# GadGadGad/Convolutional-KAN-for-Image-Classification

Hardware: AMD Instinct MI355X
Metric: images/sec fwd+bwd KAN-VGG11 3x32x32 bs=256/GPU (higher is better)
Workload: dtype f32

## Files before the change

convolutional-kan-for-image-classification_amd/_lib.py:

```python
from __future__ import annotations

import ctypes as C
import os
from typing import Optional

_HERE = os.path.dirname(os.path.abspath(__file__))
LIB_PATH = os.environ.get("KANCONV_LIB") or os.path.join(_HERE, "libkanconv.so")

KAN_MAX_PLANES = 16
KAN_MAX_TABLE = 32
KAN_FP_WORDS = 192
BASIS_BSPLINE, BASIS_RBF, BASIS_CHEBY, BASIS_POLY, BASIS_FOURIER, BASIS_RELU, BASIS_GRAM = 0, 1, 2, 3, 4, 5, 6
ACT_NONE, ACT_IDENTITY, ACT_GELU, ACT_SILU, ACT_RELU, ACT_TANH, ACT_SIGMOID, ACT_GELU_TANH = -1, 0, 1, 2, 3, 4, 5, 6


class KanGeom(C.Structure):
    _fields_ = [(n, C.c_int) for n in ("B", "C", "H", "W", "O", "Ho", "Wo", "kh", "kw", "sh", "sw", "ph", "pw", "dh", "dw", "groups")] + \
               [("x_bstride", C.c_longlong), ("y_bstride", C.c_longlong)]


class KanBasis(C.Structure):
    _fields_ = [("kind", C.c_int), ("n_basis", C.c_int), ("order", C.c_int), ("act", C.c_int),
                ("p0", C.c_float), ("p1", C.c_float), ("table", C.c_float * KAN_MAX_TABLE), ("chan_table", C.c_void_p)]


class KanPlan(C.Structure):
    _fields_ = [(n, C.c_int) for n in ("P", "K", "IPC", "KC", "Kpad", "Opad", "fwd_splits", "bwd_data_splits", "bwd_weight_splits",
                                          "fwd_target", "bwd_data_target", "bwd_weight_target", "x_pm_wanted", "dz_pm_wanted", "bwd_weight_expanded", "row_blocks", "e_pm_wanted", "fwd_expanded", "fwd_halo", "bwd_weight_halo",
                                          "fwd_band", "bwd_weight_band")] + \
               [(n, C.c_longlong) for n in ("packed_weight_bytes", "bwd_data_weight_bytes", "fwd_slab_elems", "bwd_data_slab_elems",
                                            "bwd_weight_slab_elems", "e_pm_elems")]


class KanWavGeom(C.Structure):
    _fields_ = [(n, C.c_int) for n in ("B", "C", "H", "W", "O", "Ho", "Wo", "kh", "kw", "sh", "sw", "ph", "pw", "dh", "dw", "wavelet")] + \
               [("x_bstride", C.c_longlong), ("u_bstride", C.c_longlong)]


WAVELETS = {"mexican_hat": 0, "morlet": 1, "dog": 2, "meyer": 3, "shannon": 4}

_P, _I, _LL, _F, _D = C.c_void_p, C.c_int, C.c_longlong, C.c_float, C.c_double
_GP, _BP = C.POINTER(KanGeom), C.POINTER(KanBasis)
SIGNATURES = {
    "kan_version": (C.c_char_p, []),
    "kan_last_error": (C.c_char_p, []),
    "kan_plan": (_I, [_GP, _BP, C.POINTER(KanPlan)]),
    "kan_pack_weights": (_I, [_P, _P, _P, _P, _GP, _BP, _P]),
    "kan_pack_cacheable": (_I, [_GP, _BP]),
    "kan_pack_weights_cached": (_I, [_P, _P, _P, _P, _GP, _BP, _P, _I, _I, _I, _P]),
    "kan_conv_fwd": (_I, [_P, _P, _P, _P, _GP, _BP, _P, _P]),
    "kan_position_major": (_I, [_P, _P, _I, _I, _I, _LL, _P]),
    "kan_conv_bwd_data": (_I, [_P, _P, _P, _P, _P, _P, _GP, _BP, _P, _P]),
    "kan_conv_bwd_data_params": (_I, [_P, _P, _P, _P, _P, _P, _P, _GP, _BP, _P, _P]),
    "kan_conv_bwd_weight": (_I, [_P, _P, _P, _P, _GP, _BP, _P, _P, _P]),
    "kan_position_major_expanded": (_I, [_P, _P, _GP, _BP, _P]),
    "kan_conv_fwd_expanded": (_I, [_P, _P, _P, _GP, _BP, _P]),
    "kan_conv_bwd_weight_expanded": (_I, [_P, _P, _P, _GP, _BP, _P]),
    "kan_unpack_wgrad": (_I, [_P, _P, _P, _GP, _BP, _P]),
    "kan_slab_reduce": (_I, [_P, _I, _LL, _P, _I, _I, _I, _LL, _P]),
    "kan_instnorm_prelu_fwd": (_I, [_P, _I, _LL, _P, _P, _P, _P, _P, _P, _P, _I, _I, _I, _LL, _F, _I, _P]),
    "kan_instnorm_prelu_bwd": (_I, [_P, _P, _P, _P, _P, _P, _P, _P, _P, _P, _P, _I, _I, _I, _LL, _I, _P]),
    "kan_instnorm_prelu_pool_fwd": (_I, [_P, _I, _LL, _P, _P, _P, _P, _P, _P, _P, _P, _I, _I, _I, _I, _LL, _F, _I, _P]),
    "kan_instnorm_prelu_pool_bwd": (_I, [_P, _P, _P, _P, _P, _P, _P, _P, _P, _P, _P, _P, _I, _I, _I, _I, _LL, _I, _P]),
    "kan_instnorm_prelu_poolk_fwd": (_I, [_P, _I, _LL, _P, _P, _P, _P, _P, _P, _P, _P, _I, _I, _I, _I, _LL, _F, _I, _I, _I, _P]),
    "kan_instnorm_prelu_poolk_bwd": (_I, [_P, _P, _P, _P, _P, _P, _P, _P, _P, _P, _P, _P, _I, _I, _I, _I, _LL, _I, _I, _I, _P]),
    "kan_split_supported": (_I, [C.POINTER(KanGeom), C.POINTER(KanBasis)]),
    "kan_split_weight_bytes": (_LL, [C.POINTER(KanGeom), C.POINTER(KanBasis)]),
    "kan_split_pack_weights": (_I, [_P, _P, _P, C.POINTER(KanGeom), C.POINTER(KanBasis), _P]),
    "kan_conv_fwd_split": (_I, [_P, _P, _P, C.POINTER(KanGeom), C.POINTER(KanBasis), _P]),
    "kan_wav_fwd": (_I, [_P, _P, _P, _P, _P, C.POINTER(KanWavGeom), _P]),
    "kan_wav_bwd_input": (_I, [_P, _P, _P, _P, _P, _P, C.POINTER(KanWavGeom), _P]),
    "kan_wav_param_workspace": (_LL, [C.POINTER(KanWavGeom)]),
    "kan_wav_bwd_params": (_I, [_P, _P, _P, _P, _P, _P, _P, _P, _P, C.POINTER(KanWavGeom), _P]),
    "kan_adamw_step": (_I, [_P, _P, _P, _P, _LL, _D, _D, _D, _D, _D, _I, _F, _P]),
    "kan_adamw_step_segments": (_I, [_P, _P, _P, _P, _P, _P, _P, _P, _P, _I, _I, _D, _D, _D, _D, _D, _I, _F, _P]),
}

_lib: Optional[C.CDLL] = None

# ... 29 lines not shown
```

convolutional-kan-for-image-classification_amd/csrc/kan_internal.h:

```cpp
#pragma once
#include <type_traits>
#include "kanconv.h"

int kan_fail_msg(const char* fmt, const char* a);
int kan_raise_lds_limit(const void* kernel, int bytes);

enum : int {
    FAST_GENERIC = 0,
    FAST_BSPLINE_SILU = 1,
    FAST_BSPLINE_GELU = 2,
    FAST_RBF8 = 3,
    FAST_CHEBY5 = 4,
    FAST_CHEBY4 = 5,
    FAST_POLY4 = 6,
    FAST_POLY3 = 7,
    FAST_RBF5 = 8,
    FAST_RELU8 = 9,
    FAST_GRAM4 = 10,
    FAST_POLY1 = 11,
    FAST_LAST = 11
};
enum : unsigned {
    ON_TAP_MAJOR = 1u << 0,
    ON_BIG_TILES = 1u << 1,
    ON_HALO_FWD = 1u << 2,
    ON_HALO_BWD_WEIGHT = 1u << 3,
    ON_BAND_FWD = 1u << 4,
    ON_BAND_BWD_WEIGHT = 1u << 5,
    ON_EXPANDED_FWD = 1u << 6,
    ON_EXPANDED = 1u << 7,
    ON_ROWBLK_BWD_DATA = 1u << 8,
};
struct FastSpec {
    int kind, planes;
    bool base;
    bool xn_fwd, xn_bwd;
    int kc;
    unsigned routes;
};
constexpr FastSpec fast_spec(int f) {
    constexpr unsigned bspline = ON_TAP_MAJOR | ON_BIG_TILES | ON_HALO_FWD | ON_HALO_BWD_WEIGHT | ON_BAND_FWD | ON_BAND_BWD_WEIGHT |
                                 ON_EXPANDED_FWD | ON_EXPANDED | ON_ROWBLK_BWD_DATA;
    switch (f) {
        case FAST_BSPLINE_SILU: case FAST_BSPLINE_GELU: return {KAN_BASIS_BSPLINE, 9, true, false, false, 18, bspline};
        case FAST_RBF8: return {KAN_BASIS_RBF, 9, true, true, true, 18, ON_TAP_MAJOR | ON_BAND_FWD | ON_BAND_BWD_WEIGHT};
        case FAST_RBF5: return {KAN_BASIS_RBF, 6, true, true, true, 18, ON_TAP_MAJOR};
        case FAST_CHEBY5: return {KAN_BASIS_CHEBY, 5, false, false, false, 16, ON_TAP_MAJOR | ON_BIG_TILES | ON_BAND_FWD | ON_BAND_BWD_WEIGHT};
        case FAST_CHEBY4: return {KAN_BASIS_CHEBY, 4, false, false, false, 16, ON_TAP_MAJOR | ON_HALO_FWD | ON_BAND_FWD};
        case FAST_POLY4: return {KAN_BASIS_POLY, 5, true, true, false, 16, ON_TAP_MAJOR | ON_BIG_TILES | ON_HALO_FWD | ON_BAND_FWD};
        case FAST_POLY3: return {KAN_BASIS_POLY, 4, true, true, false, 16, ON_TAP_MAJOR};
        case FAST_POLY1: return {KAN_BASIS_POLY, 2, true, true, false, 16, ON_TAP_MAJOR};
        case FAST_RELU8: return {KAN_BASIS_RELU, 9, true, false, false, 16, ON_HALO_FWD | ON_HALO_BWD_WEIGHT | ON_EXPANDED_FWD | ON_EXPANDED};
        case FAST_GRAM4: return {KAN_BASIS_GRAM, 5, true, false, false, 16, ON_HALO_FWD | ON_HALO_BWD_WEIGHT | ON_EXPANDED};
        default: return {-1, 0, false, true, true, 0, 0};
    }
}
constexpr int fast_kind(int f) { return fast_spec(f).kind; }
constexpr int fast_planes(int f) { return fast_spec(f).planes; }
constexpr bool fast_has(int f, unsigned routes) { return (fast_spec(f).routes & routes) == routes && f != FAST_GENERIC; }

template <int V> using IC = std::integral_constant<int, V>;
template <unsigned ROUTES, int F = 1, class Fn>
bool dispatch_fast(int f, Fn&& fn) {
    if constexpr (F > FAST_LAST) {
        return false;
    } else {
        if constexpr (fast_has(F, ROUTES)) {
            if (f == F) { fn(IC<F>{}); return true; }
        }
        return dispatch_fast<ROUTES, F + 1>(f, fn);
    }
}
template <int V, int... REST, class Fn>
void pick(int v, Fn&& fn) {
    if constexpr (sizeof...(REST) == 0) fn(IC<V>{});
// ... 21 lines not shown
    int lds_bytes, wgs_per_cu;
    int fwd_splits;
    int bw_ok, bw_WR, bw_NI, bw_NT, bw_tiles_o, bw_row_tiles, bw_TPI, bw_ptiles, bw_cells, bw_slots, bw_lds_bytes, bw_splits;
    unsigned short bw_ph_rt0[KAN_BAND_MAX_PHASES + 1];
    unsigned char ph_a[KAN_BAND_MAX_PHASES], ph_b[KAN_BAND_MAX_PHASES];
    short ph_tap0[KAN_BAND_MAX_PHASES + 1];
    unsigned short tap_shift[KAN_BAND_MAX_TAPS];
    unsigned short tap_rt[KAN_BAND_MAX_TAPS];
    short tap_step[KAN_BAND_MAX_TAPS], tap_nt[KAN_BAND_MAX_TAPS];
} KanBandCfg;

void kan_band_cfg(const KanGeom* g, const KanBasis* b, int fast, KanBandCfg* cfg);
int kan_band_bwd_weight_launch(const float* dz, const float* x, const float* xn, float* dwp, const KanGeom* g, const KanBasis* b,
                               const KanBandCfg* cfg, int splits, long long slab_elems, void* stream);
int kan_band_fwd_launch(const float* x, const float* xn, const float* wp, float* z, const KanGeom* g, const KanBasis* b,
                        const KanBandCfg* cfg, int splits, long long slab_elems, void* stream);

constexpr int DW_T = 9;
constexpr int DW_MAX_TP = 96;

enum class Route { TAP_MAJOR, DW, BAND, HALO, EXPANDED };

struct FwdCfg { int TO, TP, tiles_o, tiles_p, chunks, splits, slots; };
struct BdCfg { int CH, tiles_c, tiles_p, n_ob, Opad32, chunks, splits; };
struct BwCfg { int TR, TO, tiles_r, tiles_o, chunks, splits, slots; };
struct BwHaloCfg { int R, nimg, spb, n_bands, tiles_r, tiles_o, splits, bands_per_split; };

struct ConvPlan {
    KanPlan pub;
    int fast;
    Route fwd, bwd_data, bwd_weight;
    bool pm_fwd, pm_bwd_data, pm_bwd_weight;
    bool rowblk_bwd_data;
    bool pmdma_xcd, pm_lpt, pm_xcd;
    FwdCfg fc;
    BdCfg bd;
    BwCfg bw;
    BwHaloCfg bwh;
    KanBandCfg band;
};
int plan_conv(const KanGeom* g, const KanBasis* b, ConvPlan* cp);

int live_taps_out(const KanGeom* g, int hw);
int live_taps_in(const KanGeom* g, int hw);
int live_positions_for_tap(const KanGeom* g, int tap);
int balance_tiles(const int* weight, int n, unsigned short* idx);
```

convolutional-kan-for-image-classification_amd/csrc/kan_plan.hip:

```cpp
#include <hip/hip_runtime.h>
#include <cstdio>
#include <cstdlib>
#include <cstring>
#include "kanconv.h"
#include "kan_device.h"
#include "kan_common.h"
#include "kan_internal.h"

namespace {

int fail(const char* msg) { return kan_fail_msg("%s", msg); }

int check(const KanGeom* g, const KanBasis* b) {
    if (!g || !b) return fail("null geometry/basis");
    if (g->groups < 0 || g->groups > 65535) return fail("groups out of range");
    if (g->B <= 0 || g->C <= 0 || g->O <= 0 || g->H <= 0 || g->W <= 0 || g->Ho <= 0 || g->Wo <= 0) return fail("non-positive dimension");
    if (g->kh <= 0 || g->kw <= 0 || g->sh <= 0 || g->sw <= 0 || g->dh <= 0 || g->dw <= 0 || g->ph < 0 || g->pw < 0) return fail("bad conv parameters");
    if (g->kh > 255 || g->kw > 255 || g->C > 65535) return fail("kernel size / channel count out of supported range");
    if ((g->H + 2 * g->ph - g->dh * (g->kh - 1) - 1) / g->sh + 1 != g->Ho || (g->W + 2 * g->pw - g->dw * (g->kw - 1) - 1) / g->sw + 1 != g->Wo)
        return fail("Ho/Wo inconsistent with H/W, kernel, stride, padding, dilation");
    if ((long long)g->B * g->Ho * g->Wo >= (1ll << 31) || (long long)g->B * g->H * g->W >= (1ll << 31)) return fail("pixel count exceeds int32");
    if ((long long)g->B * g->x_bstride * 4 >= (1ll << 31) || (long long)g->B * g->y_bstride * 4 >= (1ll << 31))
        return fail("activation tensors must be smaller than 2 GiB (32-bit buffer offsets)");
    if (g->x_bstride < (long long)ngroups(g) * g->C * g->H * g->W || g->y_bstride < (long long)ngroups(g) * g->O * g->Ho * g->Wo)
// ... 94 lines not shown
    if (g->kh != 3 || g->kw != 3 || g->sh != 1 || g->sw != 1 || g->dh != 1 || g->dw != 1 || g->ph != 1 || g->pw != 1) return false;
    if ((g->C & 1) || g->O % 128 != 0) return false;
    if (pm_fwd) return false;
    const int W = g->W, H = g->H;
    return (W == 32 && H % 4 == 0) || (W == 16 && H % 8 == 0) || (W == 8 && H == 8) || (W == 4 && H == 4);
}
bool band_fwd(const KanGeom* g, const KanBasis* b, int f, bool dw, bool pm_fwd, bool halo, KanBandCfg* out) {
    if (tuning_off("KAN_BAND") || !fast_has(f, ON_BAND_FWD)) return false;
    if (b->kind == KAN_BASIS_POLY && b->order == 0) return false;
    if (dw || pm_fwd || halo) return false;
    if (!(g->C <= 3 || round_up(g->O, 64) % 128 != 0 || (g->kh * g->kw >= 4 && g->C % 2 == 0 && !tuning_off("KAN_BAND_WIDE")))) return false;
    kan_band_cfg(g, b, f, out);
    return out->ok != 0;
}
FwdCfg fwd_cfg(const KanGeom* g, const KanPlan& pl, bool big, bool pm_fwd, bool halo) {
    FwdCfg c;
    c.TO = (big && !pm_fwd) ? 256 : (pl.Opad % 128 == 0) ? 128 : 64;
    c.slots = c.TO == 256 ? 512 : 1024;
    c.TP = 128;
    c.tiles_o = pl.Opad / c.TO;
    c.tiles_p = ceil_div((long long)g->B * g->Ho * g->Wo, c.TP);
    c.chunks = pl.Kpad / pl.KC;
    c.splits = pick_splits((long long)c.tiles_o * c.tiles_p * ngroups(g), c.chunks, 8, 4.0 * g->B * g->O * g->Ho * g->Wo * ngroups(g), c.slots);
    if (halo) {
        const int n_pairs = g->C / 2, pps = ceil_div(n_pairs, c.splits < n_pairs ? c.splits : n_pairs);
        c.splits = ceil_div(n_pairs, pps);
    }
    return c;
}
bool rowblk_bwd_data(const KanGeom* g, int f, bool pm_bwd_data) {
    return !tuning_off("KAN_BD_ROWBLK") && fast_has(f, ON_ROWBLK_BWD_DATA) && !pm_bwd_data && g->H == 4 && g->W == 4 && g->Ho == 4 && g->Wo == 4 &&
           g->kh == 3 && g->kw == 3 && g->sh == 1 && g->sw == 1 && g->ph == 1 && g->pw == 1 && g->dh == 1 && g->dw == 1 && g->B % 8 == 0 && g->O % 16 == 0;
}
struct LiveClass { long long tiles; int live_steps; };

int pick_target_steps(const LiveClass* cls, int ncls, int min_steps, double slab_bytes, int* max_splits, long long SLOTS = 1024) {
    int hi = 1;
    for (int i = 0; i < ncls; ++i) if (cls[i].live_steps > hi) hi = cls[i].live_steps;
    int best = hi; double best_cost = -1; int best_ms = 1;
    for (int t = min_steps < hi ? min_steps : hi; t <= hi; ++t) {
        long long wgs = 0; int ms = 1;
        for (int i = 0; i < ncls; ++i) {
            const int sp = cls[i].live_steps > 0 ? ceil_div(cls[i].live_steps, t) : 1;
            wgs += cls[i].tiles * sp;
            if (sp > ms) ms = sp;
        }
        const long long rounds = (wgs + SLOTS - 1) / SLOTS;
        const double cost = (double)(rounds * (t + 6)) + ms * slab_cost_steps(slab_bytes);
        if (best_cost < 0 || cost < best_cost) { best_cost = cost; best = t; best_ms = ms; }
    }
    *max_splits = best_ms;
    return best;
}
BdCfg bd_cfg(const KanGeom* g, const KanPlan& pl) {
    BdCfg c;
    c.CH = 64 / pl.P;
    c.tiles_c = ceil_div(g->C, 2 * c.CH);
    c.tiles_p = ceil_div((long long)g->B * g->H * g->W, 128);
    c.n_ob = ceil_div(g->O, 16);
    c.Opad32 = round_up(g->O, 32);
    c.chunks = g->kh * g->kw * c.n_ob;
    c.splits = pick_splits((long long)c.tiles_c * c.tiles_p * ngroups(g), c.chunks, 8, 4.0 * g->B * g->C * g->H * g->W * ngroups(g));
    return c;
}
bool pmdma_bwd_weight(const KanGeom* g, const KanBasis* b, int f, bool want_pm_bw) {
    if (tuning_off("KAN_PMDMA") || !fast_has(f, ON_EXPANDED)) return false;
// ... 98 lines not shown
        order[j] = v;
    }
    for (int r = 0; r < n; ++r) {
        const int depth = r / 8, k = r % 8, bin = (depth & 1) ? 7 - k : k;
        int slot = depth * 8 + bin;
        if (slot >= n) slot = r;
        idx[slot] = (unsigned short)order[r];
    }
    bool seen[PERM_MAX] = {false};
    for (int i = 0; i < n; ++i) { if (idx[i] >= n || seen[idx[i]]) return 0; seen[idx[i]] = true; }
    return n;
}

int plan_conv(const KanGeom* g, const KanBasis* b, ConvPlan* cp) {
    if (int rc = check(g, b)) return rc;
    ConvPlan& c = *cp;
    KanPlan* pl = &c.pub;
    const int T = g->kh * g->kw, G = ngroups(g), f = fast_variant(b);
    c.fast = f;
    const bool pm_shape = pmdma_fwd_shape(g, f);
    c.pm_fwd = want_pix_major(g, b, PM_FWD, pm_shape);
    c.pm_bwd_data = want_pix_major(g, b, PM_BWD_DATA, false);
    const bool want_pm_bw = want_pix_major(g, b, PM_BWD_WEIGHT, false);
    const bool dw = dw_direct(g, b);
    const bool halo = halo_fwd(g, b, f, c.pm_fwd);
    c.band.ok = c.band.bw_ok = 0;
    const bool band = band_fwd(g, b, f, dw, c.pm_fwd, halo, &c.band);
    const bool pmdma_fwd = pm_shape && c.pm_fwd;
    const bool pmdma_bw = pmdma_bwd_weight(g, b, f, want_pm_bw);
    const bool halo_bw = halo_bwd_weight(g, f, pmdma_bw);
    c.pm_bwd_weight = want_pm_bw && !halo_bw;
    const bool band_bw = band && c.band.bw_ok && !want_pm_bw && !tuning_off("KAN_BAND_BW");
    c.rowblk_bwd_data = rowblk_bwd_data(g, f, c.pm_bwd_data);
    c.pmdma_xcd = tuning_on("KAN_PMDMA_XCD");
    c.pm_lpt = !tuning_off("KAN_PM_LPT");
    c.pm_xcd = !tuning_off("KAN_PM_XCD");
    c.fwd = dw ? Route::DW : band ? Route::BAND : halo ? Route::HALO : pmdma_fwd ? Route::EXPANDED : Route::TAP_MAJOR;
    c.bwd_data = dw ? Route::DW : Route::TAP_MAJOR;
    c.bwd_weight = dw ? Route::DW : band_bw ? Route::BAND : halo_bw ? Route::HALO : pmdma_bw ? Route::EXPANDED : Route::TAP_MAJOR;
    pl->P = b->n_basis + (b->act != KAN_ACT_NONE);
    pl->K = g->C * T * pl->P;
    {
        int i18 = 18 / pl->P, i16 = 16 / pl->P;
        if (i18 > 4) i18 = 4;
        if (i16 > 4) i16 = 4;
        const bool use18 = (long long)i18 * pl->P * 16 > (long long)i16 * pl->P * 18;
        pl->KC = use18 ? 18 : 16;
        pl->IPC = use18 ? i18 : i16;
        if (pl->P >= 10 && pl->P <= 12) { pl->KC = 12; pl->IPC = 1; }
        if (halo) { pl->KC = 2 * pl->P; pl->IPC = 2; }
    }
    pl->Kpad = ceil_div(g->C * T, pl->IPC) * pl->KC;
    if (band) { pl->KC = c.band.NPLE; pl->IPC = c.band.NG; pl->Kpad = c.band.n_steps * c.band.NPLE; }
    pl->Opad = round_up(g->O, 64);
    pl->packed_weight_bytes = (long long)G * pl->Kpad * pl->Opad * 4;
    c.bd = bd_cfg(g, *pl);
    pl->bwd_data_weight_bytes = (long long)G * T * c.bd.Opad32 * c.bd.tiles_c * 128 * 4;
    pl->fwd_slab_elems = (long long)g->B * g->y_bstride;
    pl->bwd_data_slab_elems = (long long)g->B * g->x_bstride;
    pl->bwd_weight_slab_elems = (long long)G * pl->K * pl->Opad;
    const bool big = big_tiles(f, *pl);
    c.fc = fwd_cfg(g, *pl, big, c.pm_fwd, halo);
    c.bw = bw_cfg(g, *pl, big, c.pm_bwd_weight);
    if (halo_bw) c.bwh = bw_halo_cfg(g, *pl);
    pl->fwd_splits = band ? c.band.fwd_splits : c.fc.splits;
    pl->bwd_data_splits = c.bd.splits;
// ... 45 lines not shown
```

convolutional-kan-for-image-classification_amd/csrc/kanconv.hip:

```cpp
#include <hip/hip_runtime.h>
#include <cstdio>
#include <cstdlib>
#include <cstring>
#include <cmath>
#include <cstdint>
#include <mutex>
#include <type_traits>
#include <vector>
#include "kanconv.h"
#include "kan_device.h"

#include "kan_common.h"
#include "kan_internal.h"

namespace {


thread_local char g_err[512] = "";
int fail(const char* fmt, const char* a = "") {
    snprintf(g_err, sizeof(g_err), fmt, a);
    return -1;
}
}
int kan_fail_msg(const char* fmt, const char* a) { return fail(fmt, a); }
// ... 557 lines not shown
            for (int r = 0; r < 16; ++r) {
                const int o = o_tile0 + w_o * 64 + mi * 32 + mfma_row(r, lane);
                if (o < g.O) zb[(size_t)o * HoWo] = acc[mi][ni][r];
            }
        }
    }
}

template <int M>
__device__ __forceinline__ void wave_reduce_scatter(float (&v)[M], int lane, int& idx, float& tot) {
    int base = 0;
    int m = M;
#pragma unroll
    for (int off = 32; off >= 1; off >>= 1) {
        if (m > 1) {
            const int h = m / 2;
            const bool up = (lane & off) != 0;
#pragma unroll
            for (int i = 0; i < M / 2; ++i) {
                if (i < h) {
                    const float keep = up ? v[h + i] : v[i], send = up ? v[i] : v[h + i];
                    v[i] = keep + __shfl_xor(send, off, 64);
                }
            }
            base += up ? h : 0;
            m = h;
        } else {
            v[0] += __shfl_xor(v[0], off, 64);
        }
    }
    idx = base; tot = v[0];
}

template <int KIND, int FAST, int RB = 0>
__global__ __launch_bounds__(256, 4) void k_conv_bwd_data(
    const float* __restrict__ dz, const float* __restrict__ x, const float* __restrict__ xn, const float* __restrict__ wd,
    float* __restrict__ dx, float* __restrict__ dxn, DevGeom g, DevBasis bs, int CH, int n_ct, int n_ob, int Opad16,
    int n_chunks, int chunks_per_split, long long slab_elems, unsigned dz_bytes, TilePerm perm, float* __restrict__ dpar) {
    constexpr int TP = 128, KD = 16, NT = 256;
    __shared__ __attribute__((aligned(16))) float smem[2 * 2 * KD * 128];
    __shared__ float sTab[KAN_MAX_TABLE];

    const int tid = threadIdx.x, lane = tid & 63;
    const int wave = __builtin_amdgcn_readfirstlane(tid >> 6);
    const int w_r = wave >> 1, w_p = wave & 1;
    const int HoWo = g.Ho * g.Wo, HW = g.H * g.W, P = bs.P;
    const int Min = g.B * HW;
    const BlockId blk = xcd_block_order(false);
    const int grp = blk.y / n_ct;
    const int px_tile0 = (perm.n ? (int)perm.idx[blk.x] : blk.x) * TP, ct = blk.y - grp * n_ct;
    const int ncol = n_ct * 128;
    const int pxl = (wave & 1) * 64 + lane, ol0 = wave >> 1;
    const bool idle_rows = (ct * 2 + w_r) * CH >= g.C;
    {
        const size_t xo = (size_t)grp * g.C * HW;
        x += xo; xn += xo; dx += xo; if (dxn) dxn += xo;
        dz += (size_t)grp * g.O * HoWo * (g.pix_major ? g.B : 1);
        wd += (size_t)grp * (g.kh * g.kw) * Opad16 * ncol;
    }

    if (tid < KAN_MAX_TABLE) sTab[tid] = bs.tab[tid];
    const int my_px = px_tile0 + (RB ? ((pxl >> 2) & 7) * 16 + (pxl >> 5) * 4 + (pxl & 3) : pxl);
    const bool pv = my_px < Min;
    int pb, ph_, pw_;
    {
        int hw;
        if (g.pix_major) { hw = my_px / g.B; pb = my_px - hw * g.B; }
        else { pb = my_px / HW; hw = my_px - pb * HW; }
        ph_ = hw / g.W; pw_ = hw - ph_ * g.W;
    }
    const kan_rsrc dz_rs = make_rsrc(dz, dz_bytes);
    const unsigned dz_img = g.pix_major ? (unsigned)pb : (unsigned)pb * (unsigned)g.ybs;
    const unsigned zstride = g.pix_major ? (unsigned)g.B : 1u;
// ... 86 lines not shown
    for (int a = 0; a < 2; ++a)
#pragma unroll
        for (int b = 0; b < 2; ++b)
#pragma unroll
            for (int r = 0; r < 16; ++r) acc[a][b][r] = 0.f;

    int ch0 = blk.z * chunks_per_split;
    int ch1 = min(n_chunks, ch0 + chunks_per_split);
    unsigned tapmask = 0xffffffffu;
    if (g.pix_major) {
        tapmask = 0;
        const int T = g.kh * g.kw;
        const int hwA = px_tile0 / g.B, hwB = min(px_tile0 + TP - 1, Min - 1) / g.B;
        for (int hw = hwA; hw <= hwB; ++hw)
            for (int tap = 0; tap < T; ++tap) tapmask |= (tap_alive_in(g, hw, tap) ? 1u : 0u) << tap;
        auto seg = [&](int tap) { return tap * n_ob; };
        const int L = live_step_count(tapmask, T, n_chunks, seg);
        const int S = min((int)gridDim.z, max(1, (L + chunks_per_split - 1) / chunks_per_split));
        if (blk.z >= S) { ch0 = ch1 = n_chunks; }
        else {
            ch0 = blk.z == 0 ? 0 : live_step_pos(tapmask, T, n_chunks, (int)((long long)L * blk.z / S), seg);
            ch1 = blk.z == S - 1 ? n_chunks : live_step_pos(tapmask, T, n_chunks, (int)((long long)L * (blk.z + 1) / S), seg);
        }
    }
    auto next_live = [&](int ch) -> int {
        if (!g.pix_major) return ch;
        while (ch < ch1) {
            const int tap = ch / n_ob;
            if ((tapmask >> tap) & 1u) return ch;
            ch = (tap + 1) * n_ob;
        }
        return ch1;
    };
    int ch = next_live(ch0);
    if (ch < ch1) { if (RB) issue_rb(ch, 0); else issue(ch, 0); }
    const int ar = w_r * 64 + (lane & 31), bp = w_p * 64 + (lane & 31), kh2 = lane >> 5;
    for (int cur = 0; ch < ch1; cur ^= 1) {
        asm volatile("s_waitcnt vmcnt(0)" ::: "memory");
        __syncthreads();
        const bool mixed_now = pend_mixed;
        ch = next_live(ch + 1);
        if (ch < ch1) { if (RB) issue_rb(ch, cur ^ 1); else issue(ch, cur ^ 1); }
        const float* cW = smem + cur * (2 * KD * 128);
        const float* cG = cW + KD * 128;
        const unsigned aw = lds_addr(cW + kh2 * 128 + ar), ag = lds_addr(cG + kh2 * TP + bp);
        if (RB) {
            const bool l0b = !(mixed_now && w_p == 0), l1a = !(mixed_now && w_p == 1);
            if (!idle_rows) KAN_MFMA_STEP_LIVE(KD / 2, aw, 128, ag, TP, true, l0b, l1a, true);
        } else if (!idle_rows) KAN_MFMA_STEP(KD / 2, aw, 128, ag, TP);
    }

    const bool same_in = (x == xn);
    const bool split_out = (dxn != nullptr);
    float* dxs = dx + (size_t)blk.z * slab_elems;
    float* dxns = split_out ? dxn + (size_t)blk.z * slab_elems : nullptr;
#define KAN_G_TO_LDS(half)                                                                                                 \
    __syncthreads();                                                                                                       \
    if (w_r == (half)) {                                                                                                   \
        _Pragma("unroll") for (int mi = 0; mi < 2; ++mi)                                                                   \
            _Pragma("unroll") for (int ni = 0; ni < 2; ++ni)                                                               \
                _Pragma("unroll") for (int r = 0; r < 16; ++r)                                                             \
                    smem[(mi * 32 + mfma_row(r, lane)) * TP + w_p * 64 + ni * 32 + (lane & 31)] = acc[mi][ni][r];          \
    }                                                                                                                      \
    __syncthreads();
    if constexpr (FAST != 0) {
        constexpr FastSpec S = fast_spec(FAST);
        constexpr int FP = S.planes, FCH = 64 / FP, NIT = (FCH + 1) / 2, NPF = S.xn_bwd ? 1 : 2;
        float xv[NPF][NIT], nv[NIT]; unsigned ok = 0;
#define KAN_FETCH(half, slot)                                                                                              \
        _Pragma("unroll") for (int it = 0; it < NIT; ++it) {                                                                   \
            const int cl = ol0 + 2 * it, c = (ct * 2 + (half)) * FCH + cl;                                                     \
            const bool v = cl < FCH && c < g.C && pv;                                                                          \
            const size_t idx = (size_t)pb * g.xbs + (size_t)c * HW + (size_t)(ph_ * g.W + pw_);                                \
            xv[slot][it] = v ? x[idx] : 0.f;                                                                                   \
            if constexpr (S.xn_bwd) nv[it] = v ? xn[idx] : 0.f;                                                                \
            ok |= (v ? 1u : 0u) << ((slot) * NIT + it);                                                                        \
        }
        if constexpr (!S.xn_bwd) {
#pragma unroll
            for (int half = 0; half < 2; ++half) KAN_FETCH(half, half)
        }
#pragma unroll 1
// ... 1440 lines not shown
        const int t = (n & ~3) + threadIdx.x;
        if (t < n) adam1(p[t], g[t], m[t], v[t], a);
    } else {
        for (int i = threadIdx.x; i < n; i += 256) adam1(p[i], g[i], m[i], v[i], a);
    }
}

AdamArgs adam_args(double lr, double beta1, double beta2, double eps, double weight_decay, int step, float grad_scale) {
    const double bc1 = 1.0 - pow(beta1, (double)step), bc2 = 1.0 - pow(beta2, (double)step);
    AdamArgs a;
    a.decay = (float)(1.0 - lr * weight_decay);
    a.w1 = (float)(1.0 - beta1); a.b2 = (float)beta2; a.w2 = (float)(1.0 - beta2);
    a.gscale = grad_scale; a.inv_bc2_sqrt = (float)(1.0 / sqrt(bc2)); a.eps = (float)eps; a.neg_step = (float)(-lr / bc1);
    return a;
}

#include "wavkan.inc"

}

extern "C" {

const char* kan_version(void) { return "kanconv 0.5 (gfx950, fp32 MFMA 32x32x2, halo forward, 128/256-output tiles)"; }
const char* kan_last_error(void) { return g_err; }

int kan_plan(const KanGeom* geom, const KanBasis* basis, KanPlan* plan) {
    if (!plan) return fail("null plan");
    ConvPlan cp;
    if (int rc = plan_conv(geom, basis, &cp)) return rc;
    *plan = cp.pub;
    return 0;
}

static bool pack_needs_clear(const KanGeom* g, const KanPlan& pl) {
    if (pl.fwd_band) return pl.KC != pl.IPC * pl.P || g->C % pl.IPC != 0;
    return pl.KC != pl.IPC * pl.P || (g->C * g->kh * g->kw) % pl.IPC != 0;
}

static int pack_weights_impl(const float* w_base, const float* w_basis, float* wp, float* wd, const KanGeom* g, const KanBasis* b,
                             const unsigned long long* fp, int fp_cur, void* stream) {
    ConvPlan cp;
    if (int rc = plan_conv(g, b, &cp)) return rc;
    const KanPlan& pl = cp.pub;
    const int hb = b->act != KAN_ACT_NONE;
    if ((hb && !w_base) || !w_basis || !wp) return fail("null weight pointer");
    hipStream_t st = (hipStream_t)stream;
    const int T = g->kh * g->kw, NI = g->C * T, G = ngroups(g);
    const long long wp_gs = (long long)pl.Kpad * pl.Opad;
    PackGeo q = pack_geo(g, b, cp, false);
    if (fp && (pack_needs_clear(g, pl) || cp.fwd == Route::DW)) return fail("cached packing is not offered for this geometry (kan_pack_cacheable)");
    if (pl.KC != pl.IPC * pl.P || (pl.fwd_band && pack_needs_clear(g, pl))) {
        if (hipMemsetAsync(wp, 0, (size_t)pl.packed_weight_bytes, st) != hipSuccess) return fail("memset failed");
    } else if (!pl.fwd_band && NI % pl.IPC != 0) {
        if (G > 1) {
            if (hipMemsetAsync(wp, 0, (size_t)pl.packed_weight_bytes, st) != hipSuccess) return fail("memset failed");
        } else {
            size_t off = (size_t)(pl.Kpad - pl.KC) * pl.Opad;
            if (hipMemsetAsync(wp + off, 0, (size_t)pl.KC * pl.Opad * 4, st) != hipSuccess) return fail("memset failed");
        }
    }
    const int nb_base = hb ? ceil_div(g->C * T, 32) : 0;
    const int tiles_x = nb_base + ceil_div(g->C * b->n_basis * T, 32), tiles_y = pl.Opad / 32;
    const long long n_tiles = (long long)tiles_x * tiles_y;
    const long long cap = fp ? 1024 : 4096;
    dim3 grid((unsigned)(n_tiles < cap ? n_tiles : cap), 1, G);
    hipLaunchKernelGGL(k_pack, grid, dim3(256), 0, st, w_base, w_basis, wp, q, nb_base, wp_gs, tiles_x, tiles_y, fp, fp_cur);
// ... 170 lines not shown
                              const KanGeom* g, const KanBasis* b, const float* dz_pm, void* stream) {
    ConvPlan cp;
    if (int rc = plan_conv(g, b, &cp)) return rc;
    const KanPlan& pl = cp.pub;
    if (dpar && cp.bwd_data == Route::DW) return fail("kan_conv_bwd_data_params: depthwise layers take the weight-gradient route");
    if (!dz || !x || !xn || !wd || !dx) return fail("null tensor pointer");
    if ((b->kind == KAN_BASIS_RELU || b->kind == KAN_BASIS_GRAM) && !b->chan_table) return fail("ReLU / Gram bases need their device parameter table (chan_table)");
    if (!dxn && x != xn) return fail("dxn is required when xn != x");
    hipStream_t st = (hipStream_t)stream;
    if (cp.bwd_data == Route::DW) {
        DevGeom dgd = dev_geom(g); DevBasis dbd = dev_basis(b);
        dim3 grid(ceil_div((long long)g->B * g->H * g->W, 256), ngroups(g));
        dispatch_kind(b->kind, [&](auto kind) {
            hipLaunchKernelGGL((k_dw_bwd_data<decltype(kind)::value>), grid, dim3(256), 0, st, dz, x, xn, wd, dx, dxn, dgd, dbd, pl.Opad, pl.IPC, pl.KC, pl.Kpad);
        });
        return launch_ok("dw_bwd_data");
    }
    const BdCfg& c = cp.bd;
    DevGeom dg = dev_geom(g);
    dg.pix_major = (dz_pm && cp.pm_bwd_data) ? 1 : 0;
    if (dg.pix_major) dz = dz_pm;
    DevBasis db = dev_basis(b);
    if ((long long)c.tiles_c * ngroups(g) > 65535) return fail("groups * channel tiles exceed the grid limit");
    dim3 grid(c.tiles_p, c.tiles_c * ngroups(g), pl.bwd_data_splits);
    const int cps = dg.pix_major ? pl.bwd_data_target : ceil_div(c.chunks, pl.bwd_data_splits);
    TilePerm perm; perm.n = 0;
    if (dg.pix_major) perm = tile_perm(c.tiles_p, [&](int t) {
        const int hw = (int)(((long long)t * 128) / g->B);
        return ceil_div(live_taps_in(g, hw < g->H * g->W ? hw : 0) * c.n_ob, cps > 0 ? cps : 1);
    });
    const int fast = (fast_spec(cp.fast).xn_bwd ? (x != xn && dxn) : (x == xn && !dxn)) ? cp.fast : FAST_GENERIC;
    const bool rb = !dg.pix_major && cp.rowblk_bwd_data;
    const unsigned dz_bytes = (unsigned)((long long)g->B * g->y_bstride * 4);
    auto launch = [&](auto kind, auto fast, auto rbv) {
        hipLaunchKernelGGL((k_conv_bwd_data<decltype(kind)::value, decltype(fast)::value, decltype(rbv)::value>), grid, dim3(256), 0, st, dz, x, xn, wd,
                           dx, dxn, dg, db, c.CH, c.tiles_c, c.n_ob, c.Opad32, c.chunks, cps, pl.bwd_data_slab_elems, dz_bytes, perm, dpar);
    };
    const bool launched = dispatch_fast<ON_TAP_MAJOR>(fast, [&](auto fv) {
        constexpr int F = decltype(fv)::value;
        if constexpr (fast_has(F, ON_ROWBLK_BWD_DATA)) {
            if (rb) return launch(IC<fast_kind(F)>{}, fv, IC<1>{});
        }
        launch(IC<fast_kind(F)>{}, fv, IC<0>{});
    });
    if (!launched) dispatch_kind(b->kind, [&](auto kind) { launch(kind, IC<FAST_GENERIC>{}, IC<0>{}); });
    return launch_ok("conv_bwd_data");
}

int kan_conv_bwd_weight(const float* dz, const float* x, const float* xn, float* dwp, const KanGeom* g, const KanBasis* b,
                        const float* x_pm, const float* dz_pm, void* stream) {
    ConvPlan cp;
    if (int rc = plan_conv(g, b, &cp)) return rc;
    const KanPlan& pl = cp.pub;
    if (!dz || !x || !xn || !dwp) return fail("null tensor pointer");
    if ((b->kind == KAN_BASIS_RELU || b->kind == KAN_BASIS_GRAM) && !b->chan_table) return fail("ReLU / Gram bases need their device parameter table (chan_table)");
    hipStream_t st = (hipStream_t)stream;
    if (cp.bwd_weight == Route::DW) {
        DevGeom dgd = dev_geom(g); DevBasis dbd = dev_basis(b);
        dim3 grid(pl.bwd_weight_splits, ngroups(g));
        dispatch_kind(b->kind, [&](auto kind) {
            hipLaunchKernelGGL((k_dw_bwd_weight<decltype(kind)::value>), grid, dim3(256), 0, st, dz, x, xn, dwp, dgd, dbd, pl.K, pl.Opad, pl.bwd_weight_slab_elems);
        });
        return launch_ok("dw_bwd_weight");
    }
    if (cp.bwd_weight == Route::BAND) {
        if (x != xn && !fast_spec(cp.fast).xn_fwd) return fail("this basis / activation pair runs on single-input kernels: pass xn == x");
        return kan_band_bwd_weight_launch(dz, x, xn, dwp, g, b, &cp.band, pl.bwd_weight_splits, pl.bwd_weight_slab_elems, stream);
    }
    const unsigned x_bytes = (unsigned)((long long)g->B * g->x_bstride * 4), dz_bytes = (unsigned)((long long)g->B * g->y_bstride * 4);
    if (cp.bwd_weight == Route::HALO) {
        if (x != xn) return fail("internal: the channel-major weight-gradient layout needs x == xn");
        const BwHaloCfg& hc = cp.bwh;
        const DevGeom dgh = dev_geom(g); const DevBasis dbh = dev_basis(b);
        if ((long long)hc.tiles_o * ngroups(g) > 65535) return fail("groups * output tiles exceed the grid limit");
        dim3 grid(hc.tiles_r, hc.tiles_o * ngroups(g), hc.splits);
        dispatch_fast<ON_HALO_BWD_WEIGHT>(cp.fast, [&](auto fv) {
            auto launch = [&](auto w, auto r, auto nimg) {
                hipLaunchKernelGGL((k_conv_bwd_weight_halo<decltype(fv)::value, decltype(w)::value, decltype(r)::value, decltype(nimg)::value>), grid,
// ... 286 lines not shown
```

include/kanconv.h:

```cpp
#ifndef KANCONV_H
#define KANCONV_H

#ifdef __cplusplus
extern "C" {
#endif

#define KAN_MAX_PLANES 16
#define KAN_MAX_TABLE  32
#define KAN_FP_WORDS   192

enum { KAN_BASIS_BSPLINE = 0, KAN_BASIS_RBF = 1, KAN_BASIS_CHEBY = 2, KAN_BASIS_POLY = 3, KAN_BASIS_FOURIER = 4, KAN_BASIS_RELU = 5, KAN_BASIS_GRAM = 6 };
enum { KAN_ACT_NONE = -1, KAN_ACT_IDENTITY = 0, KAN_ACT_GELU = 1, KAN_ACT_SILU = 2, KAN_ACT_RELU = 3,
       KAN_ACT_TANH = 4, KAN_ACT_SIGMOID = 5, KAN_ACT_GELU_TANH = 6 };

typedef struct KanGeom {
    int B, C, H, W;
    int O, Ho, Wo;
    int kh, kw, sh, sw, ph, pw, dh, dw;
    int groups;
    long long x_bstride;
    long long y_bstride;
} KanGeom;

typedef struct KanBasis {
    int kind, n_basis, order, act;
    float p0, p1;
    float table[KAN_MAX_TABLE];
    const float* chan_table;
} KanBasis;

typedef struct KanPlan {
    int P;
    int K;
    int IPC, KC;
    int Kpad, Opad;
    int fwd_splits;
    int bwd_data_splits;
    int bwd_weight_splits;
    int fwd_target, bwd_data_target, bwd_weight_target;
    int x_pm_wanted, dz_pm_wanted;
    int bwd_weight_expanded;
    int row_blocks;
    int e_pm_wanted, fwd_expanded;
    int fwd_halo, bwd_weight_halo;
    int fwd_band, bwd_weight_band;
    long long packed_weight_bytes;
    long long bwd_data_weight_bytes;
    long long fwd_slab_elems;
    long long bwd_data_slab_elems;
    long long bwd_weight_slab_elems;
    long long e_pm_elems;
} KanPlan;

const char* kan_version(void);
const char* kan_last_error(void);

int kan_plan(const KanGeom* geom, const KanBasis* basis, KanPlan* plan);

int kan_pack_weights(const float* w_base, const float* w_basis, float* wp, float* wd,
                     const KanGeom* geom, const KanBasis* basis, void* stream);

int kan_pack_cacheable(const KanGeom* geom, const KanBasis* basis);
int kan_pack_weights_cached(const float* w_base, const float* w_basis, float* wp, float* wd,
                            const KanGeom* geom, const KanBasis* basis, unsigned long long* ring, int cur, int force,
                            int sample_stride, void* stream);

int kan_conv_fwd(const float* x, const float* xn, const float* wp, float* z,
                 const KanGeom* geom, const KanBasis* basis, const float* x_pm, void* stream);

int kan_position_major(const float* src, float* dst, int B, int Cn, int HW, long long bstride, void* stream);

int kan_conv_bwd_data(const float* dz, const float* x, const float* xn, const float* wd,
                      float* dx, float* dxn,
                      const KanGeom* geom, const KanBasis* basis, const float* dz_pm, void* stream);

int kan_conv_bwd_data_params(const float* dz, const float* x, const float* xn, const float* wd, float* dx, float* dxn, float* dparams,
                             const KanGeom* geom, const KanBasis* basis, const float* dz_pm, void* stream);

int kan_conv_bwd_weight(const float* dz, const float* x, const float* xn, float* dwp,
                        const KanGeom* geom, const KanBasis* basis, const float* x_pm, const float* dz_pm, void* stream);

int kan_position_major_expanded(const float* x, float* e_pm, const KanGeom* geom, const KanBasis* basis, void* stream);
int kan_conv_fwd_expanded(const float* e_pm, const float* wp, float* z, const KanGeom* geom, const KanBasis* basis, void* stream);
int kan_conv_bwd_weight_expanded(const float* dz_pm, const float* e_pm, float* dwp,
                                 const KanGeom* geom, const KanBasis* basis, void* stream);

int kan_unpack_wgrad(const float* dwp, float* dw_base, float* dw_basis,
                     const KanGeom* geom, const KanBasis* basis, void* stream);

int kan_slab_reduce(const float* slabs, int n_slabs, long long slab_elems, float* out,
// ... 60 lines not shown
```

Before: 17200.

## Add halo-tile LDS path for 3x3 conv backward-data on bspline layers

Adds a halo variant of the backward-data kernel for 3x3 stride-1 pad-1 convolutions on 16-wide, 8x8 and 4x4 planes. Each dz output tile plus its neighbouring rows is staged once in LDS, and every one of the nine taps reads it through shifted addresses, so the per-tap gather of dz from global memory goes away. Weights are still double-buffered through global-to-LDS copies. The cost is more shared memory per block, which may lower occupancy, plus extra kernel specialisations and zero-fill and boundary logic.

Result: no change. 17180 (-0.1%).

```diff
diff --git a/convolutional-kan-for-image-classification_amd/_lib.py b/convolutional-kan-for-image-classification_amd/_lib.py
--- a/convolutional-kan-for-image-classification_amd/_lib.py
+++ b/convolutional-kan-for-image-classification_amd/_lib.py
@@ -45,6 +45,7 @@
     "kan_version": (C.c_char_p, []),
     "kan_last_error": (C.c_char_p, []),
     "kan_plan": (_I, [_GP, _BP, C.POINTER(KanPlan)]),
+    "kan_bwd_data_variant": (_I, [_GP, _BP]),
     "kan_pack_weights": (_I, [_P, _P, _P, _P, _GP, _BP, _P]),
     "kan_pack_cacheable": (_I, [_GP, _BP]),
     "kan_pack_weights_cached": (_I, [_P, _P, _P, _P, _GP, _BP, _P, _I, _I, _I, _P]),
diff --git a/convolutional-kan-for-image-classification_amd/csrc/kan_internal.h b/convolutional-kan-for-image-classification_amd/csrc/kan_internal.h
--- a/convolutional-kan-for-image-classification_amd/csrc/kan_internal.h
+++ b/convolutional-kan-for-image-classification_amd/csrc/kan_internal.h
@@ -30,6 +30,7 @@
     ON_EXPANDED_FWD = 1u << 6,
     ON_EXPANDED = 1u << 7,
     ON_ROWBLK_BWD_DATA = 1u << 8,
+    ON_HALO_BWD_DATA = 1u << 9,
 };
 struct FastSpec {
     int kind, planes;
@@ -40,7 +41,7 @@
 };
 constexpr FastSpec fast_spec(int f) {
     constexpr unsigned bspline = ON_TAP_MAJOR | ON_BIG_TILES | ON_HALO_FWD | ON_HALO_BWD_WEIGHT | ON_BAND_FWD | ON_BAND_BWD_WEIGHT |
-                                 ON_EXPANDED_FWD | ON_EXPANDED | ON_ROWBLK_BWD_DATA;
+                                 ON_EXPANDED_FWD | ON_EXPANDED | ON_ROWBLK_BWD_DATA | ON_HALO_BWD_DATA;
     switch (f) {
         case FAST_BSPLINE_SILU: case FAST_BSPLINE_GELU: return {KAN_BASIS_BSPLINE, 9, true, false, false, 18, bspline};
         case FAST_RBF8: return {KAN_BASIS_RBF, 9, true, true, true, 18, ON_TAP_MAJOR | ON_BAND_FWD | ON_BAND_BWD_WEIGHT};
@@ -128,6 +129,7 @@
     Route fwd, bwd_data, bwd_weight;
     bool pm_fwd, pm_bwd_data, pm_bwd_weight;
     bool rowblk_bwd_data;
+    int halo_bwd_data;
     bool pmdma_xcd, pm_lpt, pm_xcd;
     FwdCfg fc;
     BdCfg bd;
diff --git a/convolutional-kan-for-image-classification_amd/csrc/kan_plan.hip b/convolutional-kan-for-image-classification_amd/csrc/kan_plan.hip
--- a/convolutional-kan-for-image-classification_amd/csrc/kan_plan.hip
+++ b/convolutional-kan-for-image-classification_amd/csrc/kan_plan.hip
@@ -150,6 +150,15 @@
     return !tuning_off("KAN_BD_ROWBLK") && fast_has(f, ON_ROWBLK_BWD_DATA) && !pm_bwd_data && g->H == 4 && g->W == 4 && g->Ho == 4 && g->Wo == 4 &&
            g->kh == 3 && g->kw == 3 && g->sh == 1 && g->sw == 1 && g->ph == 1 && g->pw == 1 && g->dh == 1 && g->dw == 1 && g->B % 8 == 0 && g->O % 16 == 0;
 }
+int halo_bwd_data(const KanGeom* g, int f, bool pm_bwd_data) {
+    if (tuning_off("KAN_HALO_BD") || !fast_has(f, ON_HALO_BWD_DATA) || pm_bwd_data) return 0;
+    if (g->kh != 3 || g->kw != 3 || g->sh != 1 || g->sw != 1 || g->dh != 1 || g->dw != 1 || g->ph != 1 || g->pw != 1) return 0;
+    if (g->O % 16 != 0) return 0;
+    if (g->W == 16 && g->H % 8 == 0) return 16;
+    if (g->W == 8 && g->H == 8) return 8;
+    if (g->W == 4 && g->H == 4) return 4;
+    return 0;
+}
 struct LiveClass { long long tiles; int live_steps; };
 
 int pick_target_steps(const LiveClass* cls, int ncls, int min_steps, double slab_bytes, int* max_splits, long long SLOTS = 1024) {
@@ -314,6 +323,7 @@
     c.pm_bwd_weight = want_pm_bw && !halo_bw;
     const bool band_bw = band && c.band.bw_ok && !want_pm_bw && !tuning_off("KAN_BAND_BW");
     c.rowblk_bwd_data = rowblk_bwd_data(g, f, c.pm_bwd_data);
+    c.halo_bwd_data = dw ? 0 : halo_bwd_data(g, f, c.pm_bwd_data);
     c.pmdma_xcd = tuning_on("KAN_PMDMA_XCD");
     c.pm_lpt = !tuning_off("KAN_PM_LPT");
     c.pm_xcd = !tuning_off("KAN_PM_XCD");
diff --git a/convolutional-kan-for-image-classification_amd/csrc/kanconv.hip b/convolutional-kan-for-image-classification_amd/csrc/kanconv.hip
--- a/convolutional-kan-for-image-classification_amd/csrc/kanconv.hip
+++ b/convolutional-kan-for-image-classification_amd/csrc/kanconv.hip
@@ -613,13 +613,44 @@
     idx = base; tot = v[0];
 }
 
-template <int KIND, int FAST, int RB = 0>
+#define KAN_MFMA_STEP_HALO(NK, addrA, LDA, b0A, b1A, b0B, b1B, HALO_, OFFB, l0a, l0b, l1a, l1b)                                     \
+    do {                                                                                                                           \
+        float fa_[2][2], fb_[2][2];                                                                                                \
+        LDS_READ4H(fa_[0][0], fa_[0][1], fb_[0][0], fb_[0][1], addrA, b0A, b1A, 0, 32 * 4, 0);                                     \
+        _Pragma("unroll") for (int kk = 0; kk < (NK); ++kk) {                                                                       \
+            const int c_ = kk & 1, n_ = c_ ^ 1;                                                                                    \
+            if (kk + 1 < (NK)) {                                                                                                   \
+                if (kk + 1 < (NK) / 2)                                                                                             \
+                    LDS_READ4H(fa_[n_][0], fa_[n_][1], fb_[n_][0], fb_[n_][1], addrA, b0A, b1A, (2 * (kk + 1)) * (LDA) * 4,        \
+                               (2 * (kk + 1)) * (LDA) * 4 + 128, (2 * (kk + 1)) * (HALO_) * 4);                                    \
+                else                                                                                                               \
+                    LDS_READ4H(fa_[n_][0], fa_[n_][1], fb_[n_][0], fb_[n_][1], addrA, b0B, b1B, (2 * (kk + 1)) * (LDA) * 4,        \
+                               (2 * (kk + 1)) * (LDA) * 4 + 128, (2 * (kk + 1 - (NK) / 2)) * (HALO_) * 4 + (OFFB));                \
+                LDS_WAIT4(fa_[c_][0], fa_[c_][1], fb_[c_][0], fb_[c_][1], 4);                                                      \
+            } else {                                                                                                               \
+                LDS_WAIT4(fa_[c_][0], fa_[c_][1], fb_[c_][0], fb_[c_][1], 0);                                                      \
+            }                                                                                                                      \
+            if (kk < (NK) / 2 ? (l0a) : (l0b)) {                                                                                   \
+                acc[0][0] = MFMA32(fa_[c_][0], fb_[c_][0], acc[0][0]);                                                             \
+                acc[1][0] = MFMA32(fa_[c_][1], fb_[c_][0], acc[1][0]);                                                             \
+            }                                                                                                                      \
+            if (kk < (NK) / 2 ? (l1a) : (l1b)) {                                                                                   \
+                acc[0][1] = MFMA32(fa_[c_][0], fb_[c_][1], acc[0][1]);                                                             \
+                acc[1][1] = MFMA32(fa_[c_][1], fb_[c_][1], acc[1][1]);                                                             \
+            }                                                                                                                      \
+        }                                                                                                                          \
+    } while (0)
+
+template <int KIND, int FAST, int RB = 0, int HZ = 0>
 __global__ __launch_bounds__(256, 4) void k_conv_bwd_data(
     const float* __restrict__ dz, const float* __restrict__ x, const float* __restrict__ xn, const float* __restrict__ wd,
     float* __restrict__ dx, float* __restrict__ dxn, DevGeom g, DevBasis bs, int CH, int n_ct, int n_ob, int Opad16,
     int n_chunks, int chunks_per_split, long long slab_elems, unsigned dz_bytes, TilePerm perm, float* __restrict__ dpar) {
     constexpr int TP = 128, KD = 16, NT = 256;
-    __shared__ __attribute__((aligned(16))) float smem[2 * 2 * KD * 128];
+    constexpr int HZR = HZ == 4 ? 4 : 8, HZN = HZ ? 128 / (HZR * HZ) : 0, HZW = HZ + 2, HZIMG = (HZR + 2) * HZW, HALO = HZN * HZIMG;
+    constexpr int SMEM = (HZ && 2 * KD * 128 + KD * HALO > 2 * 2 * KD * 128) ? 2 * KD * 128 + KD * HALO : 2 * 2 * KD * 128;
+    static_assert(!RB || HZ == 0 || HZ == 4, "row blocks: 4x4 planes");
+    __shared__ __attribute__((aligned(16))) float smem[SMEM];
     __shared__ float sTab[KAN_MAX_TABLE];
 
     const int tid = threadIdx.x, lane = tid & 63;
@@ -772,9 +803,96 @@
         }
         return ch1;
     };
+    const int ar = w_r * 64 + (lane & 31), bp = w_p * 64 + (lane & 31), kh2 = lane >> 5;
+    if constexpr (HZ != 0) {
+        float* const sHz = smem + 2 * KD * 128;
+        for (int i = tid; i < KD * HALO; i += NT) sHz[i] = 0.f;
+        const int fn = tid & 127, fpx = px_tile0 + fn;
+        const int fb = fpx / HW;
+        const unsigned voff = fpx < Min ? ((unsigned)fb * (unsigned)g.ybs + (unsigned)(fpx - fb * HW)) * 4u : KAN_OOB;
+        float* const wz = sHz + ol0 * HALO + (fn / (HZR * HZ)) * HZIMG + ((fn % (HZR * HZ)) / HZ + 1) * HZW + (fn % HZ) + 1;
+        constexpr int NBR = HZ == 16 ? 2 : 0;
+        unsigned voffn = KAN_OOB; float* wzn = sHz;
+        if constexpr (NBR != 0) {
+            const int b0 = px_tile0 / HW, h0 = (px_tile0 - b0 * HW) / HZ;
+            const int side = (lane >> 4) & 1, col = lane & 15, h = side ? h0 + HZR : h0 - 1;
+            if (b0 < g.B && h >= 0 && h < g.H) voffn = ((unsigned)b0 * (unsigned)g.ybs + (unsigned)((lane >> 5) * HoWo + h * HZ + col)) * 4u;
+            wzn = sHz + (2 * wv + (lane >> 5)) * HALO + (side ? HZR + 1 : 0) * HZW + col + 1;
+        }
+        float zv[8], zn[NBR ? NBR : 1];
+#define KAN_HZ_LOAD(ob_)                                                                                                   \
+        {                                                                                                                  \
+            const unsigned so_ = (unsigned)((ob_) * KD + ol0) * row_bytes;                                                 \
+            _Pragma("unroll") for (int jj = 0; jj < 8; ++jj)                                                               \
+                zv[jj] = __builtin_bit_cast(float, __builtin_amdgcn_raw_buffer_load_b32(dz_rs, (int)voff, (int)(so_ + (unsigned)(2 * jj) * row_bytes), 0)); \
+            _Pragma("unroll") for (int k = 0; k < NBR; ++k)                                                                \
+                zn[k] = __builtin_bit_cast(float, __builtin_amdgcn_raw_buffer_load_b32(dz_rs, (int)voffn, (int)((unsigned)((ob_) * KD + 2 * wv + 8 * k) * row_bytes), 0)); \
+        }
+#define KAN_HZ_WRITE()                                                                                                     \
+        {                                                                                                                  \
+            _Pragma("unroll") for (int jj = 0; jj < 8; ++jj) wz[2 * jj * HALO] = zv[jj];                                   \
+            _Pragma("unroll") for (int k = 0; k < NBR; ++k) wzn[8 * k * HALO] = zn[k];                                     \
+        }
+        auto issue_w = [&](int ob_, int j_, int buf) {
+            float* dW = smem + buf * (KD * 128);
+            const bool mixed = RB && j_ >= 3;
+            const int m = j_ - 3, t = m >> 1, og = m & 1;
+#pragma unroll
+            for (int q = 0; q < 2; ++q) {
+                const int blk2 = q * 4 + wv;
+                const int row = mixed ? ((blk2 < 4 ? t : 6 + t) * Opad16 + ob_ * KD + og * 8 + (blk2 & 3) * 2)
+                                      : ((RB ? 3 + j_ : j_) * Opad16 + ob_ * KD + blk2 * 2);
+                glds16((const float*)((const char*)(wd + (size_t)row * ncol + ct * 128) + wlane), dW + blk2 * 256);
+            }
+        };
+        unsigned vb[2];
+#pragma unroll
+        for (int q = 0; q < 2; ++q) {
+            const int n = w_p * 64 + q * 32 + (lane & 31);
+            int img = n / (HZR * HZ), rem = n - img * (HZR * HZ), row = rem / HZ, col = rem - row * HZ;
+            if (RB) { row = n / (HZN * HZ); rem = n - row * (HZN * HZ); img = rem / HZ; col = rem - img * HZ; }
+            vb[q] = lds_addr(sHz + kh2 * HALO + img * HZIMG + (row + 1) * HZW + (col + 1));
+        }
+        int ob = ch0 / 9, j = ch0 - ob * 9;
+        if (ch0 < ch1) { issue_w(ob, j, 0); KAN_HZ_LOAD(ob) }
+        __syncthreads();
+        if (ch0 < ch1) KAN_HZ_WRITE()
+        int buf = 0;
+#pragma unroll 1
+        for (int ch = ch0; ch < ch1; ++ch) {
+            asm volatile("s_waitcnt vmcnt(0)" ::: "memory");
+            __syncthreads();
+            int jn = j + 1, obn = ob;
+            if (jn == 9) { jn = 0; ++obn; }
+            if (ch + 1 < ch1) issue_w(obn, jn, buf ^ 1);
+            if ((j == 4 || (ch == ch0 && j > 4)) && (ob + 1) * 9 < ch1) KAN_HZ_LOAD(ob + 1)
+            const unsigned aw = lds_addr(smem + buf * (KD * 128) + kh2 * 128 + ar);
+            if constexpr (RB) {
+                const bool mixed = j >= 3;
+                const int m = j - 3, t = mixed ? (m >> 1) : j, og = m & 1;
+                const unsigned shA = mixed ? (unsigned)((HZW + 1 - t + og * 8 * HALO) * 4) : (unsigned)((1 - t) * 4);
+                const unsigned shB = mixed ? (unsigned)((1 - t - HZW + og * 8 * HALO) * 4) : (unsigned)((1 - t + 8 * HALO) * 4);
+                const unsigned a0 = vb[0] + shA, a1 = vb[1] + shA, b0 = vb[0] + shB, b1 = vb[1] + shB;
+                const bool l0b = !(mixed && w_p == 0), l1a = !(mixed && w_p == 1);
+                if (!idle_rows) KAN_MFMA_STEP_HALO(KD / 2, aw, 128, a0, a1, b0, b1, HALO, 0, true, l0b, l1a, true);
+            } else {
+                const int r = j / 3, t = j - r * 3;
+                const unsigned sh = (unsigned)(((1 - r) * HZW + (1 - t)) * 4);
+                const unsigned a0 = vb[0] + sh, a1 = vb[1] + sh;
+                if (!idle_rows) KAN_MFMA_STEP_HALO(KD / 2, aw, 128, a0, a1, a0, a1, HALO, 8 * HALO * 4, true, true, true, true);
+            }
+            if (j == 8 && ch + 1 < ch1) {
+                __syncthreads();
+                KAN_HZ_WRITE()
+            }
+            j = jn; ob = obn; buf ^= 1;
+        }
+#undef KAN_HZ_LOAD
+#undef KAN_HZ_WRITE
+    }
+    if constexpr (HZ == 0) {
     int ch = next_live(ch0);
     if (ch < ch1) { if (RB) issue_rb(ch, 0); else issue(ch, 0); }
-    const int ar = w_r * 64 + (lane & 31), bp = w_p * 64 + (lane & 31), kh2 = lane >> 5;
     for (int cur = 0; ch < ch1; cur ^= 1) {
         asm volatile("s_waitcnt vmcnt(0)" ::: "memory");
         __syncthreads();
@@ -788,6 +906,7 @@
             const bool l0b = !(mixed_now && w_p == 0), l1a = !(mixed_now && w_p == 1);
             if (!idle_rows) KAN_MFMA_STEP_LIVE(KD / 2, aw, 128, ag, TP, true, l0b, l1a, true);
         } else if (!idle_rows) KAN_MFMA_STEP(KD / 2, aw, 128, ag, TP);
+    }
     }
 
     const bool same_in = (x == xn);
@@ -2294,6 +2413,12 @@
     return 0;
 }
 
+int kan_bwd_data_variant(const KanGeom* geom, const KanBasis* basis) {
+    ConvPlan cp;
+    if (int rc = plan_conv(geom, basis, &cp)) return rc;
+    return cp.halo_bwd_data ? 1 : 0;
+}
+
 static bool pack_needs_clear(const KanGeom* g, const KanPlan& pl) {
     if (pl.fwd_band) return pl.KC != pl.IPC * pl.P || g->C % pl.IPC != 0;
     return pl.KC != pl.IPC * pl.P || (g->C * g->kh * g->kw) % pl.IPC != 0;
@@ -2530,18 +2655,22 @@
     const int fast = (fast_spec(cp.fast).xn_bwd ? (x != xn && dxn) : (x == xn && !dxn)) ? cp.fast : FAST_GENERIC;
     const bool rb = !dg.pix_major && cp.rowblk_bwd_data;
     const unsigned dz_bytes = (unsigned)((long long)g->B * g->y_bstride * 4);
-    auto launch = [&](auto kind, auto fast, auto rbv) {
-        hipLaunchKernelGGL((k_conv_bwd_data<decltype(kind)::value, decltype(fast)::value, decltype(rbv)::value>), grid, dim3(256), 0, st, dz, x, xn, wd,
-                           dx, dxn, dg, db, c.CH, c.tiles_c, c.n_ob, c.Opad32, c.chunks, cps, pl.bwd_data_slab_elems, dz_bytes, perm, dpar);
+    auto launch = [&](auto kind, auto fast, auto rbv, auto hz) {
+        hipLaunchKernelGGL((k_conv_bwd_data<decltype(kind)::value, decltype(fast)::value, decltype(rbv)::value, decltype(hz)::value>), grid, dim3(256), 0, st,
+                           dz, x, xn, wd, dx, dxn, dg, db, c.CH, c.tiles_c, c.n_ob, c.Opad32, c.chunks, cps, pl.bwd_data_slab_elems, dz_bytes, perm, dpar);
     };
     const bool launched = dispatch_fast<ON_TAP_MAJOR>(fast, [&](auto fv) {
         constexpr int F = decltype(fv)::value;
+        if constexpr (fast_has(F, ON_HALO_BWD_DATA)) {
+            if (cp.halo_bwd_data == 4 && rb) return launch(IC<fast_kind(F)>{}, fv, IC<1>{}, IC<4>{});
+            if (cp.halo_bwd_data) return pick<16, 8, 4>(cp.halo_bwd_data, [&](auto hz) { launch(IC<fast_kind(F)>{}, fv, IC<0>{}, hz); });
+        }
         if constexpr (fast_has(F, ON_ROWBLK_BWD_DATA)) {
-            if (rb) return launch(IC<fast_kind(F)>{}, fv, IC<1>{});
-        }
-        launch(IC<fast_kind(F)>{}, fv, IC<0>{});
+            if (rb) return launch(IC<fast_kind(F)>{}, fv, IC<1>{}, IC<0>{});
+        }
+        launch(IC<fast_kind(F)>{}, fv, IC<0>{}, IC<0>{});
     });
-    if (!launched) dispatch_kind(b->kind, [&](auto kind) { launch(kind, IC<FAST_GENERIC>{}, IC<0>{}); });
+    if (!launched) dispatch_kind(b->kind, [&](auto kind) { launch(kind, IC<FAST_GENERIC>{}, IC<0>{}, IC<0>{}); });
     return launch_ok("conv_bwd_data");
 }
 
diff --git a/include/kanconv.h b/include/kanconv.h
--- a/include/kanconv.h
+++ b/include/kanconv.h
@@ -56,6 +56,8 @@
 const char* kan_last_error(void);
 
 int kan_plan(const KanGeom* geom, const KanBasis* basis, KanPlan* plan);
+
+int kan_bwd_data_variant(const KanGeom* geom, const KanBasis* basis);
 
 int kan_pack_weights(const float* w_base, const float* w_basis, float* wp, float* wd,
                      const KanGeom* geom, const KanBasis* basis, void* stream);
```
